# itxtx/normalizing-flows-study

Measured on AMD Instinct MI355X. Metric: log_prob samples/sec/GPU + test-NLL match; RealNVP d=2 and MAF d=63, higher is better.
Workload: dtype fp32

## Files before the change

### normalizing-flows-study_amd/csrc/nfx_affine.hip

```cpp
#include <atomic>
#include <climits>
#include <cstdlib>

#include "nfx_affine_kernel.h"
#include "nfx_affine_small_kernel.h"
#include "nfx_pack.h"

namespace nfx {


__global__ void affine_pack_kernel(NfxMlpRaw s_net, NfxMlpRaw b_net, const float* mask, int d,
                                   int H, float* packed) {
    const int HT = (H + 31) / 32;
    const AffineLayout L = affine_layout(d, HT);
    for (int i = blockIdx.x * blockDim.x + threadIdx.x; i < L.s; i += gridDim.x * blockDim.x) {
        float v = 0.f;
        if (i >= L.mask) {
            int j = i - L.mask;
            v = j < d ? mask[j] : 0.f;
        } else {
            const int net = i / L.net;
            const NfxMlpRaw& P = net ? b_net : s_net;
            const int o = i - net * L.net;
            if (o < L.b1) {
                const RowCol e = a1_elem(o - L.w1, L.KS1);
                v = (e.row < H && e.col < d) ? mlp_weight(P, 0, d, e.row, e.col) : 0.f;
            } else if (o < L.w2) {
                int row = acc_vec_row(o - L.b1);
                v = row < H ? mlp_bias(P, 0, row) : 0.f;
            } else if (o < L.b2) {
                const ATileElem e = a_tile_elem(o - L.w2);
                int row = 32 * (e.tile / HT) + e.row, col = 32 * (e.tile % HT) + e.k;
                v = (row < H && col < H) ? mlp_weight(P, 1, H, row, col) : 0.f;
            } else if (o < L.w3) {
                int row = acc_vec_row(o - L.b2);
                v = row < H ? mlp_bias(P, 1, row) : 0.f;
            } else if (o < L.b3 && d > 8) {
                const ATileElem e = a_tile_elem(o - L.w3);
                int row = 32 * (e.tile / HT) + e.row, col = 32 * (e.tile % HT) + e.k;
                v = (row < d && col < H) ? mlp_weight(P, 2, H, row, col) : 0.f;
            } else if (o < L.b3) {
                int t = o - L.w3, j = t / (32 * HT), col = acc_vec_row(t % (32 * HT));
                v = col < H ? mlp_weight(P, 2, H, j, col) : 0.f;
            } else if (d > 8) {
                int row = acc_vec_row(o - L.b3);
                v = row < d ? mlp_bias(P, 2, row) : 0.f;
            } else {
                int j = o - L.b3;
                v = j < d ? mlp_bias(P, 2, j) : 0.f;
            }
        }
        packed[i] = v;
    }
}

__global__ __launch_bounds__(1024) void affine_split_pack_kernel(float* packed, int d, int H) {
    const int HT = (H + 31) / 32, KS1 = (d + 1) / 2;
    const AffineLayout L = affine_layout(d, HT);
    const AffineSplit S = affine_split(d, HT);
    float* out = packed + L.s;
    __shared__ int w2_bad;
    __shared__ float rowsum[2 * 64], bmax[2 * 64], w2sum[2 * 64], w3sum[2 * 8];
    if (threadIdx.x == 0) w2_bad = 0;
    __syncthreads();
    bool bad = false;
    for (int i = threadIdx.x; i < S.total; i += blockDim.x) {
        const int net = i < S.mask ? i / S.net : 0;
        const int o = i - net * S.net;
        const float* P = packed + net * L.net;
        uint32_t v = 0;
        if (i >= S.ok) {
            continue;
        } else if (i >= S.mask) {
            v = __float_as_uint(packed[L.mask + (i - S.mask)]);
        } else if (o < S.b1) {
            v = __float_as_uint(P[L.w1 + (o - S.w1)]);
        } else if (o < S.b2) {
            v = __float_as_uint(P[L.b1 + (o - S.b1)]);
        } else if (o < S.w3) {
            v = __float_as_uint(P[L.b2 + (o - S.b2)]);
        } else if (o < S.b3) {
            v = __float_as_uint(P[L.w3 + (o - S.w3)]);
        } else if (o < S.w2s) {
            v = __float_as_uint(P[L.b3 + (o - S.b3)]);
        } else {
            const int t = o - S.w2s, q = t & 3, lane = (t >> 2) & 63, g = t >> 8;
            const int p = g % 3, kb = (g / 3) % (2 * HT), hto = (g / 3) / (2 * HT);
            const int kt = kb >> 1;
            uint32_t half[2];
            for (int e = 0; e < 2; ++e) {
                const int r = 8 * (kb & 1) + 2 * q + e;
                const float w = P[L.w2 + ((hto * HT + kt) * 4 + (r >> 2)) * 256 + lane * 4 + (r & 3)];
                if (!(fabsf(w) <= 1e6f)) bad = true;
                const uint32_t u0 = __builtin_bit_cast(uint16_t, (__bf16)w);
                const float r1 = w - __uint_as_float(u0 << 16);
                const uint32_t u1 = __builtin_bit_cast(uint16_t, (__bf16)r1);
                const uint32_t u2 = __builtin_bit_cast(uint16_t, (__bf16)(r1 - __uint_as_float(u1 << 16)));
                half[e] = p == 0 ? u0 : p == 1 ? u1 : u2;
            }
            v = half[0] | (half[1] << 16);
        }
        out[i] = __uint_as_float(v);
    }
    if (bad) atomicOr(&w2_bad, 1);
    for (int i = threadIdx.x; i < 2 * 64; i += blockDim.x) {
        rowsum[i] = 0.f;
        bmax[i] = 0.f;
        w2sum[i] = 0.f;
        if (i < 2 * 8) w3sum[i] = 0.f;
    }
    __syncthreads();
    if (threadIdx.x < 2 * 32 * HT) {
        const int net = threadIdx.x / (32 * HT), row = threadIdx.x % (32 * HT), ht = row >> 5, c = row & 31;
        const float* P = packed + net * L.net;
        float sum = 0.f;
        for (int ks = 0; ks < KS1; ++ks)
            for (int hh = 0; hh < 2; ++hh) sum += fabsf(P[L.w1 + (ht * KS1 + ks) * 64 + c + 32 * hh]);
        rowsum[net * 64 + row] = sum;
        float b = 0.f;
        for (int r = 0; r < 16; ++r)
            for (int hh = 0; hh < 2; ++hh)
                if (crow(r, hh) == c) b = fabsf(P[L.b1 + ht * 32 + 16 * hh + r]);
        bmax[net * 64 + row] = b;
        float s2 = 0.f;
        for (int g = 0; g < HT * 4; ++g)
            for (int hh = 0; hh < 2; ++hh)
                for (int rr = 0; rr < 4; ++rr) s2 += fabsf(P[L.w2 + (ht * HT * 4 + g) * 256 + (c + 32 * hh) * 4 + rr]);
        w2sum[net * 64 + row] = s2;
    }
    if (threadIdx.x < 2 * d) {
        const int net = threadIdx.x / d, j = threadIdx.x % d;
        const float* P = packed + net * L.net;
        float s3 = 0.f;
        for (int t = 0; t < HT * 32; ++t) s3 += fabsf(P[L.w3 + j * HT * 32 + t]);
        w3sum[net * 8 + j] = s3;
    }
    __syncthreads();
    if (threadIdx.x == 0) {
        float n1 = 0.f, c1 = 0.f;
        bool nan = false;
        for (int i = 0; i < 2 * 64; ++i) {
            nan = nan || !(rowsum[i] <= 3e38f) || !(bmax[i] <= 3e38f);
            n1 = fmaxf(n1, rowsum[i]);
            c1 = fmaxf(c1, bmax[i]);
        }
        const float xs = nan ? 0.f : (1e30f - c1) / n1;
        bool lost = false;
        for (int net = 0; net < 2; ++net) {
            float r2 = 0.f, r3 = 0.f;
            for (int i = 0; i < 64; ++i) r2 = fmaxf(r2, w2sum[net * 64 + i]);
            for (int j = 0; j < 8; ++j) r3 = fmaxf(r3, w3sum[net * 8 + j]);
            lost = lost || !(0x1p-133 * (double)r2 * (double)r3 < 0x1p-24);
        }
        out[S.ok] = (w2_bad || lost) ? 0.f : 1.f;
        out[S.ok + 1] = xs > 0.f ? xs : 0.f;
        out[S.ok + 2] = 0.f;
        out[S.ok + 3] = 0.f;
    }
}

int affine_split_pack(float* packed, int d, int H, hipStream_t s) {
    if (!affine_has_split(d, (H + 31) / 32)) return NFX_OK;
    affine_split_pack_kernel<<<1, 1024, 0, s>>>(packed, d, H);
    return check_launch("affine_split_pack_kernel");
}

static affine_kernel_t pick_affine(int HT, int d, int dir, bool logp) {
    return pick_range<1, 4>(HT, [=](auto HT_) { return affine_pick_ht<HT_()>(d, dir, logp); });
}

static affine_kernel_t pick_affine_small(int HT, int d, int dir, bool logp) {
    return pick_range<1, 4>(HT, [=](auto HT_) { return affine_small_pick_ht<HT_()>(d, dir, logp); });
}

static std::atomic<int>& affine_policy() {
    static std::atomic<int> v{[] {
        const char* e = getenv("NFX_AFFINE_POLICY");
        return e ? atoi(e) : NFX_AFFINE_AUTO;
    }()};
    return v;
}

int affine_policy_get() { return affine_policy().load(std::memory_order_relaxed); }

typedef void (*affine_wide_t)(const float*, const float*, float*, float*, int64_t, int, int, int64_t, float*,
                              double*, double*, float);

template <int HT>
static affine_wide_t wide_pick(int dir, bool logp) {
    if (dir > 0) return affine_wide_kernel<HT, 1, false>;
    return logp ? affine_wide_kernel<HT, -1, true> : affine_wide_kernel<HT, -1, false>;
}

static int affine_wide_launch(const float* packed, const float* in, float* out, float* log_det, int64_t B, int d,
                              int H, int direction, int accumulate, float* logp, double* sums, void* workspace,
                              hipStream_t stream) {
    const bool fused = sums != nullptr;
    const int HT = (H + 31) / 32;
    if (d > 64 || HT > 4)
        return set_error(NFX_EUNSUPPORTED, "affine_coupling: d=%d H=%d outside the compiled family (d<=64, H<=128)", d, H);
    affine_wide_t k = pick_range<1, 4>(HT, [=](auto HT_) { return wide_pick<HT_()>(direction, fused); });
    if (B == 0) return fused ? gauss_finish(reinterpret_cast<double*>(workspace), 0, sums, 0, stream) : NFX_OK;
    if (!packed || !in || !out || !log_det) return set_error(NFX_EINVAL, "affine_coupling: null pointer");
    if (in == out) return set_error(NFX_EINVAL, "affine_coupling: in and out must not alias");
    const size_t lds = (size_t)kWideWaves * 32 * (d | 1) * sizeof(float);
    const int64_t ntiles = (B + 31) / 32;
    int grid = resident_grid((const void*)k, 64 * kWideWaves, lds, (ntiles + kWideWaves - 1) / kWideWaves);
    if (grid > kMaxPartials) grid = kMaxPartials;
    double* partials = reinterpret_cast<double*>(workspace);
    k<<<grid, 64 * kWideWaves, lds, stream>>>(packed, in, out, log_det, B, d, accumulate, ntiles, logp, partials,
                                              sums, gauss_const(d));
    return check_launch("affine_wide_kernel");
}

static int affine_launch(const float* packed, const float* in, float* out, float* log_det, int64_t B,
                         int d, int H, int direction, int accumulate, float* logp, double* sums,
// ... 111 lines not shown
```

### normalizing-flows-study_amd/csrc/nfx_affine_kernel.h

```cpp
#pragma once
#include <type_traits>
#include <utility>

#include "nfx_common.h"

namespace nfx {

__host__ __device__ constexpr int up4(int v) { return (v + 3) & ~3; }

struct AffineLayout {
    int d, HT, KS1;
    int w1, b1, w2, b2, w3, b3, net, mask, total;
    int s;
};

struct AffineSplit {
    int w1, b1, b2, w3, b3, w2s, net, mask, ok, total;
};

__host__ __device__ constexpr AffineSplit affine_split(int d, int HT) {
    AffineSplit S{};
    int o = 0;
    S.w1 = o; o += HT * ((d + 1) / 2) * 64;
    S.b1 = o; o += HT * 32;
    S.b2 = o; o += HT * 32;
    S.w3 = o; o += d * HT * 32;
    S.b3 = o; o += up4(d);
    S.w2s = o; o += HT * 2 * HT * 768;
    S.net = o;
    S.mask = 2 * o;
    S.ok = S.mask + up4(d);
    S.total = S.ok + 4;
    return S;
}

__host__ __device__ constexpr bool affine_has_split(int d, int HT) { return d <= 8 && HT <= 2; }

__host__ __device__ constexpr AffineLayout affine_layout(int d, int HT) {
    AffineLayout L{};
    L.d = d;
    L.HT = HT;
    L.KS1 = (d + 1) / 2;
    int o = 0;
    L.w1 = o; o += HT * L.KS1 * 64;
    L.b1 = o; o += HT * 32;
    L.w2 = o; o += HT * HT * 16 * 64;
    L.b2 = o; o += HT * 32;
    if (d <= 8) {
        L.w3 = o; o += d * HT * 32;
        L.b3 = o; o += up4(d);
    } else {
        const int NJ = (d + 31) / 32;
        L.w3 = o; o += NJ * HT * 1024;
        L.b3 = o; o += NJ * 32;
    }
    L.net = o;
    L.mask = 2 * o;
    L.total = 2 * o + up4(d);
    L.s = L.total;
    if (affine_has_split(d, HT)) L.total += affine_split(d, HT).total;
    return L;
}

template <int D>
__device__ __forceinline__ void load_row(const float* __restrict__ p, float (&v)[D]) {
    if constexpr (D == 2) {
        float2 t = *reinterpret_cast<const float2*>(p);
        v[0] = t.x; v[1] = t.y;
// ... 78 lines not shown
    for (int j = 0; j < D; ++j)
        res[j] = tclamp(halves_sum(part[j][0], part[j][1]) + P[L.b3 + j], -10.f, 10.f);
}

#ifndef NFX_SPLIT_TERMS
#define NFX_SPLIT_TERMS 6
#endif
typedef __bf16 bf16x8 __attribute__((ext_vector_type(8)));
typedef uint32_t u32x4 __attribute__((ext_vector_type(4)));

__device__ __forceinline__ f32x16 mfma_bf16(u32x4 a, u32x4 b, f32x16 c) {
    return __builtin_amdgcn_mfma_f32_32x32x16_bf16(__builtin_bit_cast(bf16x8, a), __builtin_bit_cast(bf16x8, b), c,
                                                    0, 0, 0);
}

__device__ __forceinline__ void split3(float x, uint32_t& u0, uint32_t& u1, uint32_t& u2) {
    u0 = __float_as_uint(x) & 0xffff0000u;
    const float r1 = x - __uint_as_float(u0);
    u1 = __float_as_uint(r1) & 0xffff0000u;
    u2 = __float_as_uint(r1 - __uint_as_float(u1));
}

__device__ __forceinline__ uint32_t pack_bf16(uint32_t lo, uint32_t hi) {
    return __builtin_amdgcn_perm(hi, lo, 0x07060302u);
}

__device__ __forceinline__ void split_block(const f32x16& a, int half, u32x4 (&xp)[3]) {
#pragma unroll
    for (int q = 0; q < 4; ++q) {
        uint32_t l0, l1, l2, h0, h1, h2;
        split3(a[8 * half + 2 * q], l0, l1, l2);
        split3(a[8 * half + 2 * q + 1], h0, h1, h2);
        xp[0][q] = pack_bf16(l0, h0);
        xp[1][q] = pack_bf16(l1, h1);
        xp[2][q] = pack_bf16(l2, h2);
    }
}

template <class F, int... I>
__device__ __forceinline__ void static_for_seq(F&& f, std::integer_sequence<int, I...>) {
    (f(std::integral_constant<int, I>{}), ...);
}
template <int N, class F>
__device__ __forceinline__ void static_for(F&& f) {
    static_for_seq(f, std::make_integer_sequence<int, N>{});
}

#if NFX_SPLIT_TERMS == 8
constexpr int kSplitTermW[8] = {2, 1, 2, 1, 0, 1, 0, 0}, kSplitTermX[8] = {1, 2, 0, 1, 2, 0, 1, 0};
#else
constexpr int kSplitTermW[6] = {2, 1, 0, 1, 0, 0}, kSplitTermX[6] = {0, 1, 2, 0, 1, 0};
#endif

template <int HT, int D, int TILES>
__device__ __forceinline__ void affine_nets_split_pipe(const float* __restrict__ S, const AffineSplit& SL,
                                                       const float (&xb)[2][(D + 1) / 2], float (&sv)[D],
                                                       float (&bv)[D]) {
    constexpr int KS1 = (D + 1) / 2;
    constexpr int NS = 2 * TILES;
    constexpr int KB = 2 * HT;
    constexpr int NT = NFX_SPLIT_TERMS;
    constexpr int NM = NT * HT;
    constexpr int NG = KB * NM;
    constexpr int NFI = 16 * HT;
    constexpr int NQ = 3 * HT;
    constexpr int WG0 = (NM - NQ) / 2;
    constexpr int L1G = (KB - 2) * NM;
    constexpr int L1P = L1G >= 2 ? L1G - 2 : 0;
    constexpr int HB0 = NM / 2;
    const int lane = lane_id(), h = lane >> 5;

    const float* Sn[NS];
    const u32x4* w2n[NS];
    f32x16 h1[NS][HT];
    uint32_t u[NS * KB][3][8];
    u32x4 xp[NS * KB][3];
    u32x4 w[NS * KB][HT][3];
    f32x16 hi[NS][HT], lo[NS][HT];
    f32x4 w3q[NS][HT][D][4];
    float r1[NS * KB][8], tf[NS][NFI];
    float part[2][D][2];
#pragma unroll
    for (int n = 0; n < 2; ++n)
#pragma unroll
        for (int j = 0; j < D; ++j) part[n][j][0] = part[n][j][1] = 0.f;

    auto base = [&](int s) __attribute__((always_inline)) {
        Sn[s] = S + (s / TILES) * SL.net + opaque_zero();
        w2n[s] = reinterpret_cast<const u32x4*>(Sn[s] + SL.w2s) + lane;
    };
    auto l1_bias = [&](int s) __attribute__((always_inline)) {
#pragma unroll
        for (int ht = 0; ht < HT; ++ht) h1[s][ht] = load_bias16(Sn[s] + SL.b1 + ht * 32, h);
    };
    auto l1_mfma = [&](int s) __attribute__((always_inline)) {
#pragma unroll
        for (int ht = 0; ht < HT; ++ht)
#pragma unroll
            for (int ks = 0; ks < KS1; ++ks)
                h1[s][ht] = mfma32(Sn[s][SL.w1 + (ht * KS1 + ks) * 64 + lane], xb[s % TILES][ks], h1[s][ht]);
    };
    auto split_slot = [&](int b, int i) __attribute__((always_inline)) {
        const int s = b / KB, kb = b % KB, q = i / 3;
#pragma unroll
        for (int e = 2 * q; e < 2 * q + 2; ++e) {
            if (i % 3 == 0) {
                const float x = trelu(h1[s][kb >> 1][8 * (kb & 1) + e]);
                u[b][0][e] = __float_as_uint(x) & 0xffff0000u;
                r1[b][e] = x - __uint_as_float(u[b][0][e]);
            } else if (i % 3 == 1) {
                u[b][1][e] = __float_as_uint(r1[b][e]) & 0xffff0000u;
                u[b][2][e] = __float_as_uint(r1[b][e] - __uint_as_float(u[b][1][e]));
            }
        }
        if (i % 3 == 2) {
#pragma unroll
            for (int p = 0; p < 3; ++p) xp[b][p][q] = pack_bf16(u[b][p][2 * q], u[b][p][2 * q + 1]);
        }
    };
    auto w2_quad = [&](int b, int i) __attribute__((always_inline)) {
        const int s = b / KB, kb = b % KB, p = 2 - i / HT, hto = i % HT;
        w[b][hto][p] = w2n[s][((hto * KB + kb) * 3 + p) * 64];
    };
    auto w3_quads = [&](int s, int hto, int rq) __attribute__((always_inline)) {
#pragma unroll
        for (int j = 0; j < D; ++j)
            w3q[s][hto][j][rq] = *reinterpret_cast<const f32x4*>(Sn[s] + SL.w3 + (j * HT + hto) * 32 + 16 * h + 4 * rq);
    };
    auto fold_relu = [&](int s, int f) __attribute__((always_inline)) {
        tf[s][f] = trelu(hi[s][f / 16][f % 16] + lo[s][f / 16][f % 16]);
    };
    auto fold_fma = [&](int s, int f) __attribute__((always_inline)) {
        const int hto = f / 16, r = f % 16;
#pragma unroll
        for (int j = 0; j < D; ++j)
            part[s / TILES][j][s % TILES] = fmaf(w3q[s][hto][j][r / 4][r % 4], tf[s][f], part[s / TILES][j][s % TILES]);
    };
    constexpr auto fold_gap = [](int f) { return (((f | 1) + 1) * NG + NFI - 1) / NFI - 1; };
    constexpr auto w3_gap = [](int f) {
        const int g = (((f | 1) + 1) * NG + NFI - 1) / NFI - 1;
        return g >= 2 ? g - 2 : 0;
    };
    static_assert(fold_gap(NFI - 1) < NG && fold_gap(0) >= 1 && w3_gap(0) < fold_gap(0), "fold schedule");
    static_assert(WG0 >= 0 && WG0 + NQ <= NM && HB0 + HT <= NM - HT, "read schedule");
    static_assert(KB < 2 || L1G <= (KB - 1) * NM - 1, "layer 1 of the next stage precedes its first split");

    base(0);
    l1_bias(0);
#pragma unroll
    for (int i = 0; i < NQ; ++i) w2_quad(0, i);
    l1_mfma(0);
#pragma unroll
    for (int i = 0; i < 12; ++i) split_slot(0, i);

    static_for<NS>([&](auto sc) __attribute__((always_inline)) {
        constexpr int s = decltype(sc)::value;
        static_for<NG>([&](auto gc) __attribute__((always_inline)) {
            constexpr int g = decltype(gc)::value;
            constexpr int kb = g / NM, m = g % NM, b = s * KB + kb;
            constexpr int t = m / HT, hto = m % HT;
            __builtin_amdgcn_sched_barrier(0);
            if (t == NT - 1) {
                hi[s][hto] = mfma_bf16(w[b][hto][kSplitTermW[t]], xp[b][kSplitTermX[t]], hi[s][hto]);
            } else {
                lo[s][hto] = mfma_bf16(w[b][hto][kSplitTermW[t]], xp[b][kSplitTermX[t]],
                                       kb == 0 && t == 0 ? f32x16{} : lo[s][hto]);
            }
            __builtin_amdgcn_sched_barrier(0);
            if (g == 0 && s + 1 < NS) base(s + 1);
            if (b + 1 < NS * KB && m >= WG0 && m < WG0 + NQ) w2_quad(b + 1, m - WG0);
            if (kb == 0 && m >= HB0 && m < HB0 + HT)
                hi[s][m - HB0] = load_bias16(Sn[s] + SL.b2 + (m - HB0) * 32, h);
            if (s > 0) {
#pragma unroll
                for (int fq = 0; fq < NFI; fq += 4)
                    if (w3_gap(fq) == g) w3_quads(s - 1, fq / 16, (fq % 16) / 4);
            }
            if (s + 1 < NS && g == L1P) l1_bias(s + 1);
            if (s + 1 < NS && g == L1G) l1_mfma(s + 1);
            if (b + 1 < NS * KB) {
#pragma unroll
                for (int i = m * 12 / NM; i < (m + 1) * 12 / NM; ++i) split_slot(b + 1, i);
            }
            if (s > 0) {
#pragma unroll
                for (int f = 0; f < NFI; ++f)
                    if ((fold_gap(f) >= 1 ? fold_gap(f) - 1 : 0) == g) fold_relu(s - 1, f);
#pragma unroll
                for (int f = 0; f < NFI; ++f)
                    if (fold_gap(f) == g) fold_fma(s - 1, f);
            }
        });
    });
    __builtin_amdgcn_sched_barrier(0);
#pragma unroll
    for (int fq = 0; fq < NFI; fq += 4) w3_quads(NS - 1, fq / 16, (fq % 16) / 4);
#pragma unroll
    for (int f = 0; f < NFI; ++f) {
        fold_relu(NS - 1, f);
        fold_fma(NS - 1, f);
    }
#pragma unroll
    for (int j = 0; j < D; ++j) {
        sv[j] = tclamp(halves_sum(part[0][j][0], part[0][j][1]) + Sn[0][SL.b3 + j], -10.f, 10.f);
        bv[j] = tclamp(halves_sum(part[1][j][0], part[1][j][1]) + Sn[NS - 1][SL.b3 + j], -10.f, 10.f);
    }
}

template <int HT, int D, int TILES = 2>
__device__ __forceinline__ void affine_net_split(const float* __restrict__ S, const AffineSplit& SL,
                                                 const float (&xb)[2][(D + 1) / 2], float (&res)[D]) {
    constexpr int KS1 = (D + 1) / 2;
    const int lane = lane_id(), h = lane >> 5;

    f32x16 h1[HT][2];
#pragma unroll
    for (int ht = 0; ht < HT; ++ht) {
        f32x16 a0, a1;
        load_bias16_x2(S + SL.b1 + ht * 32, h, a0, a1);
#pragma unroll
        for (int ks = 0; ks < KS1; ++ks) {
            const float w = S[SL.w1 + (ht * KS1 + ks) * 64 + lane];
            a0 = mfma32(w, xb[0][ks], a0);
            if constexpr (TILES == 2) a1 = mfma32(w, xb[1][ks], a1);
        }
#pragma unroll
        for (int r = 0; r < 16; ++r) {
            a0[r] = trelu(a0[r]);
            if constexpr (TILES == 2) a1[r] = trelu(a1[r]);
        }
        h1[ht][0] = a0;
        h1[ht][1] = a1;
    }

    float part[D][2];
#pragma unroll
    for (int j = 0; j < D; ++j) part[j][0] = part[j][1] = 0.f;
    auto fold = [&](int hto, const f32x16& a, int st) {
#pragma unroll
        for (int j = 0; j < D; ++j) {
            const f32x16 w3 = load_bias16(S + SL.w3 + (j * HT + hto) * 32, h);
#pragma unroll
            for (int r = 0; r < 16; ++r) part[j][st] = fmaf(w3[r], trelu(a[r]), part[j][st]);
        }
    };
    const u32x4* w2s = reinterpret_cast<const u32x4*>(S + SL.w2s) + lane;
#pragma unroll
    for (int st = 0; st < TILES; ++st) {
        u32x4 xp[2 * HT][3];
#pragma unroll
        for (int kb = 0; kb < 2 * HT; ++kb) split_block(h1[kb >> 1][st], kb & 1, xp[kb]);
        const u32x4* w2 = w2s + opaque_zero();
#pragma unroll
        for (int hto = 0; hto < HT; ++hto) {
            f32x16 hi = load_bias16(S + SL.b2 + hto * 32 + opaque_zero(), h), lo = {};
#pragma unroll
            for (int kb = 0; kb < 2 * HT; ++kb) {
                const int g = (hto * 2 * HT + kb) * 3;
                const u32x4 w[3] = {w2[g * 64], w2[(g + 1) * 64], w2[(g + 2) * 64]};
#if NFX_SPLIT_TERMS == 8
                lo = mfma_bf16(w[2], xp[kb][1], lo);
                lo = mfma_bf16(w[1], xp[kb][2], lo);
#endif
                lo = mfma_bf16(w[2], xp[kb][0], lo);
                lo = mfma_bf16(w[1], xp[kb][1], lo);
                lo = mfma_bf16(w[0], xp[kb][2], lo);
                lo = mfma_bf16(w[1], xp[kb][0], lo);
                lo = mfma_bf16(w[0], xp[kb][1], lo);
                hi = mfma_bf16(w[0], xp[kb][0], hi);
            }
            fold(hto, hi + lo, st);
        }
    }
#pragma unroll
    for (int j = 0; j < D; ++j)
        res[j] = tclamp(halves_sum(part[j][0], part[j][1]) + S[SL.b3 + j], -10.f, 10.f);
}

__host__ __device__ constexpr bool affine_split_piped(int HT, int D) { return HT == 2 && D <= 4; }

template <int HT, int D, int TILES, bool PIPE>
__device__ __forceinline__ void affine_nets_split(const float* __restrict__ S, const AffineSplit& SL,
                                                  const float* __restrict__ Pg, const AffineLayout& L,
                                                  const float (&xb)[2][(D + 1) / 2], float (&sv)[D], float (&bv)[D]) {
    constexpr int KS1 = (D + 1) / 2;
    const bool wok = S[SL.ok] != 0.f;
    const float xs = S[SL.ok + 1];
    bool fast[2];
#pragma unroll
    for (int st = 0; st < 2; ++st) {
        bool bad = false;
#pragma unroll
        for (int ks = 0; ks < KS1; ++ks) bad = bad || !(fabsf(xb[st][ks]) <= xs);
        fast[st] = wok && __builtin_amdgcn_ballot_w64(bad) == 0;
    }
    if constexpr (PIPE) {
        affine_nets_split_pipe<HT, D, TILES>(S, SL, xb, sv, bv);
    } else {
        affine_net_split<HT, D, TILES>(S, SL, xb, sv);
        __builtin_amdgcn_sched_barrier(0);
        affine_net_split<HT, D, TILES>(S + SL.net, SL, xb, bv);
    }
    if (!(fast[0] && (TILES == 1 || fast[1]))) {
        __builtin_amdgcn_sched_barrier(0);
        const float* P = Pg + opaque_zero();
        float s2[D], b2[D];
        affine_net<HT, D, TILES>(P, L, xb, s2);
        __builtin_amdgcn_sched_barrier(0);
        affine_net<HT, D, TILES>(P + L.net, L, xb, b2);
        if (!fast[lane_id() >> 5]) {
#pragma unroll
            for (int j = 0; j < D; ++j) {
                sv[j] = s2[j];
                bv[j] = b2[j];
            }
        }
    }
}

template <int HT, int D, int DIR, bool LOGP>
__global__ __launch_bounds__(256) void affine_coupling_kernel(
    const float* __restrict__ packed, const float* __restrict__ in, float* __restrict__ out,
    float* __restrict__ logdet, int64_t B, int accumulate, int64_t nchunks,
    float* __restrict__ logp, double* __restrict__ partials, double* __restrict__ sums, float cgauss) {
    constexpr AffineLayout L = affine_layout(D, HT);
    constexpr int KS1 = L.KS1;
    constexpr bool SPLIT = affine_has_split(D, HT);
    constexpr AffineSplit SL = affine_split(D, HT);
    constexpr int MASK = SPLIT ? SL.mask : L.mask;
    extern __shared__ f32x4 lds4[];
    {
        const f32x4* src = reinterpret_cast<const f32x4*>(packed + (SPLIT ? L.s : 0));
        for (int i = threadIdx.x; i < (SPLIT ? SL.total : L.total) / 4; i += 256) lds4[i] = src[i];
    }
    __syncthreads();
    const float* sm = reinterpret_cast<const float*>(lds4);

    const int lane = lane_id(), h = lane >> 5, col = lane & 31;
    const int64_t nwaves = (int64_t)gridDim.x * 4;
    float mk[D], mkb[KS1];
#pragma unroll
    for (int j = 0; j < D; ++j) mk[j] = sm[MASK + j];
#pragma unroll
    for (int ks = 0; ks < KS1; ++ks) mkb[ks] = (2 * ks + h < D) ? sm[MASK + 2 * ks + h] : 0.f;

    const int64_t wv = (int64_t)blockIdx.x * 4 + (threadIdx.x >> 6);
    const int64_t F = nchunks / nwaves, R = nchunks - F * nwaves;
    const bool split = 2 * R <= nwaves;
    const int64_t nfull = split ? F : F + (wv < R ? 1 : 0);
    const bool half = split && wv < 2 * R;
    const int64_t half_base = F * nwaves * 64 + wv * 32;

    struct Fetch {
        float xb[2][KS1];
        float xr[D];
        float ldin;
    };
    auto fetch = [&](int64_t u, Fetch& f) {
        const int64_t base = u < nfull ? (wv + u * nwaves) * 64 : half_base;
        const int nsamp = u < nfull ? 64 : (u == nfull && half ? 32 : 0);
#pragma unroll
        for (int st = 0; st < 2; ++st) {
            const int64_t s = base + 32 * st + col;
#pragma unroll
            for (int ks = 0; ks < KS1; ++ks) {
                const int k = 2 * ks + h;
                f.xb[st][ks] = (32 * st + col < nsamp && k < D && s < B) ? in[s * D + k] : 0.f;
            }
        }
        const int64_t so = base + lane;
        if (lane < nsamp && so < B) {
            load_row<D>(in + so * D, f.xr);
            f.ldin = accumulate ? logdet[so] : 0.f;
        } else {
#pragma unroll
            for (int j = 0; j < D; ++j) f.xr[j] = 0.f;
            f.ldin = 0.f;
        }
    };

    double lpacc = 0.0;
    auto unit = [&](auto tiles_c, int64_t base, const Fetch& cur) {
        constexpr int TILES = decltype(tiles_c)::value;
        const float* smi = sm + opaque_zero();
        float xb[2][KS1];
#pragma unroll
        for (int st = 0; st < 2; ++st) {
#pragma unroll
            for (int ks = 0; ks < KS1; ++ks) xb[st][ks] = cur.xb[st][ks] * mkb[ks];
        }

        float sv[D], bv[D];
        if constexpr (SPLIT) {
            affine_nets_split<HT, D, TILES, false>(smi, SL, packed, L, xb, sv, bv);
        } else {
            affine_net<HT, D, TILES>(smi, L, xb, sv);
            affine_net<HT, D, TILES>(smi + L.net, L, xb, bv);
        }
// ... 203 lines not shown
```

### normalizing-flows-study_amd/csrc/nfx_affine_schain.hip

```cpp
#include "nfx_chain.h"

namespace nfx {

template <int HT, int D>
__host__ __device__ constexpr int schain_wpad() {
    return (affine_split(D, HT).total + 255) & ~255;
}

template <int HT, int D, int DIR, bool LOGP, int NW>
__global__ __launch_bounds__(64 * NW) void affine_schain_kernel(
    NfxChainPacks packs, int nl, const float* __restrict__ in, float* __restrict__ out,
    float* __restrict__ logdet, int64_t B, int accumulate, int64_t nchunks, int slice_chunks,
    float* __restrict__ logp, double* __restrict__ partials, double* __restrict__ sums, float cgauss) {
    constexpr AffineLayout L = affine_layout(D, HT);
    constexpr AffineSplit SL = affine_split(D, HT);
    static_assert(affine_has_split(D, HT), "the streaming chain runs the split nets");
    constexpr int KS1 = L.KS1;
    constexpr int WPAD = schain_wpad<HT, D>();
    constexpr int NT = 64 * NW;
    extern __shared__ f32x4 lds4[];
    float* wbuf = reinterpret_cast<float*>(lds4);
    float* sx = wbuf + 2 * WPAD;
    float* sld = sx + (size_t)slice_chunks * 64 * D;

    const uint32_t wbuf_lds = lds_addr_of(lds4);
    const int wave = __builtin_amdgcn_readfirstlane(threadIdx.x >> 6);
    const int lane = lane_id(), h = lane >> 5, col = lane & 31;
    const int64_t c0 = nchunks * blockIdx.x / gridDim.x, c1 = nchunks * (blockIdx.x + 1) / gridDim.x;

    auto stage = [&](int li, int buf) {
        const float* src = packs.p[DIR > 0 ? li : nl - 1 - li] + L.s;
        for (int c = wave; c < WPAD / 256; c += NW) {
            int idx = c * 256 + lane * 4;
            if (idx > SL.total - 4) idx = SL.total - 4;
            lds_dma_x4(src + idx, wbuf_lds + (uint32_t)(buf * WPAD + c * 256) * 4u);
        }
    };

    double lpacc = 0.0;
    int g = 0;
    if (c0 < c1) stage(0, 0);
    for (int64_t s0 = c0; s0 < c1; s0 += slice_chunks) {
        const int64_t s1 = s0 + slice_chunks < c1 ? s0 + slice_chunks : c1;
        const int64_t r0 = s0 * 64;
        const int rows = (int)((B < s1 * 64 ? B : s1 * 64) - r0);
        for (int e = threadIdx.x; e < rows * D; e += NT) sx[e] = in[r0 * D + e];
        for (int e = threadIdx.x; e < rows; e += NT) sld[e] = accumulate ? logdet[r0 + e] : 0.f;
        const int nch = (int)(s1 - s0);
        const int F = nch / NW, R = nch - F * NW;
        const bool split = 2 * R <= NW;
        const int nfull = split ? F : F + (wave < R ? 1 : 0);
        const bool half = split && wave < 2 * R;
        const int half_base = F * NW * 64 + wave * 32;

        for (int li = 0; li < nl; ++li) {
            lds_dma_wait();
            __syncthreads();
            if (li + 1 < nl)
                stage(li + 1, (g + 1) & 1);
            else if (s0 + slice_chunks < c1)
                stage(0, (g + 1) & 1);
            const float* W = wbuf + (g & 1) * WPAD;
            const float* Pg = packs.p[DIR > 0 ? li : nl - 1 - li];
            const bool first = li == 0 && !accumulate;
            float mk[D], mkb[KS1];
#pragma unroll
            for (int j = 0; j < D; ++j) mk[j] = W[SL.mask + j];
#pragma unroll
            for (int ks = 0; ks < KS1; ++ks) mkb[ks] = (2 * ks + h < D) ? W[SL.mask + 2 * ks + h] : 0.f;

            auto unit = [&](auto tiles_c, int ub) {
                constexpr int TILES = decltype(tiles_c)::value;
                const int so = ub + lane;
                const bool act = lane < 32 * TILES && so < rows;
                float xr[D];
                if (act) {
                    load_row<D>(sx + so * D, xr);
                } else {
#pragma unroll
                    for (int j = 0; j < D; ++j) xr[j] = 0.f;
                }
                float xb[2][KS1];
                if constexpr (D == 2) {
                    const float other = halves_other(xr[0], xr[1]);
                    xb[0][0] = (h ? other : xr[0]) * mkb[0];
                    xb[1][0] = (h ? xr[1] : other) * mkb[0];
                } else {
#pragma unroll
                    for (int st = 0; st < 2; ++st) {
                        const int s = ub + 32 * st + col;
#pragma unroll
                        for (int ks = 0; ks < KS1; ++ks) {
                            const int k = 2 * ks + h;
                            xb[st][ks] = (32 * st + col < 32 * TILES && s < rows && k < D) ? sx[s * D + k] * mkb[ks] : 0.f;
                        }
                    }
                }
                const float* Wi = W + opaque_zero();
                float sv[D], bv[D];
                affine_nets_split<HT, D, TILES, affine_split_piped(HT, D)>(Wi, SL, Pg, L, xb, sv, bv);
                if (act) {
#pragma clang fp contract(off)
                    float y[D];
                    float ld = 0.f;
#pragma unroll
                    for (int j = 0; j < D; ++j) {
                        const float m = mk[j], om = 1.f - m;
                        const float xa = xr[j] * m;
                        float t;
                        if constexpr (DIR < 0) {
                            t = (xr[j] - bv[j]) * exp_fast(-sv[j]);
                            ld = ld + om * (-sv[j]);
                        } else {
                            t = xr[j] * exp_fast(sv[j]) + bv[j];
                            ld = ld + om * sv[j];
                        }
                        const float v = xa + om * t;
                        y[j] = nonfinite(v) ? 0.f : v;
                    }
                    if (nonfinite(ld)) ld = 0.f;
                    store_row<D>(sx + so * D, y);
                    sld[so] = first ? ld : sld[so] + ld;
                }
            };
            for (int u = 0; u < nfull; ++u) unit(std::integral_constant<int, 2>{}, (wave + u * NW) * 64);
            if (half) unit(std::integral_constant<int, 1>{}, half_base);
            ++g;
        }
        __syncthreads();
        for (int e = threadIdx.x; e < rows * D; e += NT) out[r0 * D + e] = sx[e];
        for (int e = threadIdx.x; e < rows; e += NT) {
            const float ldt = sld[e];
            logdet[r0 + e] = ldt;
            if constexpr (LOGP) {
                const float* rw = sx + (size_t)e * D;
                float m = gauss_sq0(rw[0]);
#pragma unroll
                for (int j = 1; j < D; ++j) m = gauss_sq(m, rw[j]);
                const float lp = gauss_lp(m, cgauss, ldt);
                logp[r0 + e] = lp;
                lpacc += (double)lp;
            }
        }
        __syncthreads();
    }
    if constexpr (LOGP) {
        logp_commit<NT>(lpacc, partials, sums, B);
    }
}

typedef void (*schain_t)(NfxChainPacks, int, const float*, float*, float*, int64_t, int, int64_t, int, float*,
                         double*, double*, float);

__host__ __device__ constexpr int schain_waves(int HT, int D) { return affine_split_piped(HT, D) ? 8 : 12; }

template <int HT, int D>
static schain_t schain_pick_d(int dir, bool logp) {
    constexpr int NW = schain_waves(HT, D);
    if (dir > 0) return affine_schain_kernel<HT, D, 1, false, NW>;
    return logp ? affine_schain_kernel<HT, D, -1, true, NW> : affine_schain_kernel<HT, D, -1, false, NW>;
}

static schain_t schain_pick(int HT, int D, int dir, bool logp) {
    if (HT == 1) return D == 2 ? schain_pick_d<1, 2>(dir, logp) : D == 4 ? schain_pick_d<1, 4>(dir, logp) : schain_pick_d<1, 8>(dir, logp);
    if (HT == 2) return D == 2 ? schain_pick_d<2, 2>(dir, logp) : D == 4 ? schain_pick_d<2, 4>(dir, logp) : schain_pick_d<2, 8>(dir, logp);
    return nullptr;
}

static int schain_wpad_rt(int HT, int D) {
    return (affine_split(D, HT).total + 255) & ~255;
}

constexpr size_t kSchainLds = 160 * 1024;
constexpr size_t kSchainStatic = 1024;

static int64_t schain_slice_cap(int HT, int D) {
    const size_t w = 2 * (size_t)schain_wpad_rt(HT, D) * sizeof(float);
    if (w + kSchainStatic >= kSchainLds) return 0;
    return (int64_t)((kSchainLds - kSchainStatic - w) / (64 * (D + 1) * sizeof(float)));
// ... 34 lines not shown
```

### normalizing-flows-study_amd/csrc/nfx_chain.h

```cpp
#pragma once
#include "nfx_affine_kernel.h"
#include "nfx_rng.h"

namespace nfx {

constexpr int kChainMax = 64;
struct NfxChainPacks {
    const float* p[kChainMax];
};

__device__ __forceinline__ void lds_dma_x4(const float* src, uint32_t lds_addr) {
    const uint32_t m = lds_addr;
    uint32_t keep;
    asm volatile(
        "s_mov_b32 %0, m0\n\t"
        "s_mov_b32 m0, %2\n\t"
        "s_nop 0\n\t"
        "global_load_lds_dwordx4 %1, off\n\t"
        "s_mov_b32 m0, %0"
        : "=&s"(keep)
        : "v"(src), "s"(__builtin_amdgcn_readfirstlane(m))
        : "memory");
}
template <typename T>
__device__ __forceinline__ uint32_t lds_addr_of(T* shared_array) {
    return (uint32_t)(uintptr_t)((__attribute__((address_space(3))) T*)shared_array);
}
__device__ __forceinline__ void lds_dma_wait() { asm volatile("s_waitcnt vmcnt(0)" ::: "memory"); }


int schain_launch(const NfxChainPacks& P, int nl, const float* in, float* out, float* log_det, int64_t B, int d,
                  int H, int direction, int accumulate, float* logp, double* sums, void* workspace, hipStream_t s);
bool schain_supported(int64_t B, int d, int H);
int affine_policy_get();
constexpr int64_t kSmallChainMaxB = 1 << 16;

}
```

### normalizing-flows-study_amd/csrc/nfx_spline_schain_kernel.h

```cpp
#pragma once
#include "nfx_chain.h"
#include "nfx_spline_kernel.h"

namespace nfx {

template <int HT>
__host__ __device__ constexpr int spline_schain_wpad() {
    return (spline_layout(HT, 2).total + 255) & ~255;
}

template <int HT, int K, int DIR, bool LOGP, int NW>
__global__ __launch_bounds__(64 * NW) void spline_schain_kernel(
    NfxChainPacks packs, int nl, const float* __restrict__ in, float* __restrict__ out,
    float* __restrict__ logdet, int64_t B, SplineConsts C, int accumulate, int64_t nchunks, int slice_chunks,
    float* __restrict__ logp, double* __restrict__ partials, double* __restrict__ sums, float cgauss,
    uint64_t seed, uint64_t* rng, float* __restrict__ zout) {
#pragma clang fp contract(off)
    constexpr int D = 2;
    constexpr SplineLayout L = spline_layout(HT, D);
    constexpr int WPAD = spline_schain_wpad<HT>();
    constexpr int NTH = 64 * NW;
    extern __shared__ f32x4 lds4[];
    float* wbuf = reinterpret_cast<float*>(lds4);
    float* sx = wbuf + 2 * WPAD;
    float* sld = sx + (size_t)slice_chunks * 64 * D;

    const uint32_t wbuf_lds = lds_addr_of(lds4);
    const int wave = __builtin_amdgcn_readfirstlane(threadIdx.x >> 6);
    const int lane = lane_id(), h = lane >> 5;
    const int64_t c0 = nchunks * blockIdx.x / gridDim.x, c1 = nchunks * (blockIdx.x + 1) / gridDim.x;

    auto stage = [&](int li, int buf) {
        const float* src = packs.p[DIR > 0 ? li : nl - 1 - li];
        for (int c = wave; c < WPAD / 256; c += NW) {
            int idx = c * 256 + lane * 4;
            if (idx > L.total - 4) idx = L.total - 4;
            lds_dma_x4(src + idx, wbuf_lds + (uint32_t)(buf * WPAD + c * 256) * 4u);
        }
    };

#ifdef NFX_SCHAIN_TIMING
    long long tacc[6] = {0, 0, 0, 0, 0, 0};
    long long tmark = clock64();
#define NFX_CMARK(k) do { const long long t_ = clock64(); tacc[k] += t_ - tmark; tmark = t_; } while (0)
#else
#define NFX_CMARK(k) do { } while (0)
#endif
    double lpacc = 0.0;
    int g = 0;
    if (c0 < c1) stage(0, 0);
    for (int64_t s0 = c0; s0 < c1; s0 += slice_chunks) {
        const int64_t s1 = s0 + slice_chunks < c1 ? s0 + slice_chunks : c1;
        const int64_t r0 = s0 * 64;
        const int rows = (int)((B < s1 * 64 ? B : s1 * 64) - r0);
        if (rng) {
            const uint64_t off = rng_offset(rng);
            for (int e = threadIdx.x; e < rows; e += NTH) {
                float z[D];
                base_draw<D>(r0 + e, seed, off, z);
                sx[e * D] = z[0];
                sx[e * D + 1] = z[1];
                if (zout) {
                    zout[(r0 + e) * D] = z[0];
                    zout[(r0 + e) * D + 1] = z[1];
                }
            }
        } else {
            for (int e = threadIdx.x; e < rows * D; e += NTH) sx[e] = in[r0 * D + e];
        }
        for (int e = threadIdx.x; e < rows; e += NTH) sld[e] = accumulate ? logdet[r0 + e] : 0.f;
        const int nch = (int)(s1 - s0);
        const int F = nch / NW, R = nch - F * NW;
        const bool split = 2 * R <= NW;
        const int nfull = split ? F : F + (wave < R ? 1 : 0);
        const bool half = split && wave < 2 * R;
        const int half_base = F * NW * 64 + wave * 32;

        NFX_CMARK(4);
        for (int li = 0; li < nl; ++li) {
            NFX_CMARK(3);
            lds_dma_wait();
            __syncthreads();
            NFX_CMARK(0);
            if (li + 1 < nl)
                stage(li + 1, (g + 1) & 1);
            else if (s0 + slice_chunks < c1)
                stage(0, (g + 1) & 1);
            const float* W = wbuf + (g & 1) * WPAD;
            const bool first = li == 0 && !accumulate;
            const int NT = (int)W[L.meta];
            const float mkb = h < D ? W[L.mask + h] : 0.f;

            auto unit = [&](auto tiles_c, int ub) {
                constexpr int TILES = decltype(tiles_c)::value;
                const int so = ub + lane;
                const bool act = lane < 32 * TILES && so < rows;
                float xr[D];
                if (act) {
                    const f32x2 v = *reinterpret_cast<const f32x2*>(sx + so * D);
                    xr[0] = v.x;
                    xr[1] = v.y;
                } else {
                    xr[0] = xr[1] = 0.f;
                }
                float xb[2][4];
                {
                    const float other = halves_other(xr[0], xr[1]);
                    float xraw[2] = {h ? other : xr[0], h ? xr[1] : other};
#pragma unroll
                    for (int st = 0; st < 2; ++st) {
                        float xv = xraw[st];
                        if (C.rescale) xv = C.rs_to_scale * (xv - C.rs_lo) - C.bound;
                        xb[st][0] = xv * mkb;
                        xb[st][1] = xb[st][2] = xb[st][3] = 0.f;
                    }
                }
                float y[D];
                float ld;
#ifdef NFX_SCHAIN_TIMING
                {
                    const float* Wz = W + opaque_zero();
                    f32x16 h2[HT][2];
                    spline_unit_hidden<HT, TILES>(Wz, L, 1, xb, h2);
                    float prm[32];
                    spline_unit_params<HT, TILES>(Wz, L, h2, 0, prm);
                    NFX_CMARK(1);
#pragma unroll
                    for (int j = 0; j < D; ++j) y[j] = xr[j];
                    ld = 0.f;
                    spline_unit_dim<K, DIR, D>(C, (int)Wz[L.tdim], 0, prm, xr, y, ld);
                    NFX_CMARK(2);
                }
#else
                if constexpr (NW > 8 && HT > 1)
                    spline_unit_apply_tseq<HT, K, DIR, D, TILES>(W + opaque_zero(), L, C, 1, NT, xb, xr, y, ld);
                else
                    spline_unit_apply<HT, K, DIR, D, TILES>(W + opaque_zero(), L, C, 1, NT, xb, xr, y, ld);
#endif
                if (act) {
                    float yo[D];
#pragma unroll
                    for (int j = 0; j < D; ++j) yo[j] = nonfinite(y[j]) ? 0.f : y[j];
                    *reinterpret_cast<f32x2*>(sx + so * D) = f32x2{yo[0], yo[1]};
                    if (nonfinite(ld)) ld = 0.f;
                    sld[so] = first ? ld : sld[so] + ld;
                }
            };
            for (int u = 0; u < nfull; ++u) unit(std::integral_constant<int, 2>{}, (wave + u * NW) * 64);
            if (half) unit(std::integral_constant<int, 1>{}, half_base);
            ++g;
        }
        NFX_CMARK(3);
        __syncthreads();
        for (int e = threadIdx.x; e < rows * D; e += NTH) out[r0 * D + e] = sx[e];
        for (int e = threadIdx.x; e < rows; e += NTH) {
            const float ldt = sld[e];
            logdet[r0 + e] = ldt;
            if constexpr (LOGP) {
                const float* rw = sx + (size_t)e * D;
                const float m = gauss_sq(gauss_sq0(rw[0]), rw[1]);
                const float lp = gauss_lp(m, cgauss, ldt);
                logp[r0 + e] = lp;
                lpacc += (double)lp;
            }
        }
        __syncthreads();
    }
    NFX_CMARK(5);
#ifdef NFX_SCHAIN_TIMING
    if (blockIdx.x == 0 && lane == 0 && (wave == 0 || wave == 4))
        for (int k = 0; k < 6; ++k) out[(wave ? 6 : 0) + k] = (float)tacc[k];
#endif
    if constexpr (LOGP) {
        logp_commit<NTH>(lpacc, partials, sums, B);
    }
    if (rng) rng_commit(rng);
}

typedef void (*spline_schain_t)(NfxChainPacks, int, const float*, float*, float*, int64_t, SplineConsts, int, int64_t,
                                int, float*, double*, double*, float, uint64_t, uint64_t*, float*);

constexpr int kSplineSchainWaves = 12;
constexpr int kSplineSchainWavesSmall = 8;

template <int HT>
spline_schain_t spline_schain_pick_ht(int K, int dir, bool logp, bool small);

template <int HT, int K, int NW>
spline_schain_t spline_schain_dir(int dir, bool logp) {
    if (dir > 0) return spline_schain_kernel<HT, K, 1, false, NW>;
    return logp ? spline_schain_kernel<HT, K, -1, true, NW> : spline_schain_kernel<HT, K, -1, false, NW>;
}

template <int HT>
spline_schain_t spline_schain_pick(int K, int dir, bool logp, bool small) {
    return pick_range<kSplineMinK, kSplineMaxK>(K, [=](auto K_) {
        return small ? spline_schain_dir<HT, K_(), kSplineSchainWavesSmall>(dir, logp)
                     : spline_schain_dir<HT, K_(), kSplineSchainWaves>(dir, logp);
    });
}

}
// ... 1 lines not shown
```

Measured before the change: 1.578 billion.

## Elide masked-out output rows in affine split pipe and rebalance chain tiles per SIMD

The pack kernel now detects which coupling-layer outputs are masked (their s/b are discarded) and, when numerically safe, records a compact list of live output indices. The piped split-net kernel then computes only the live half of the final-layer outputs, which cuts w3 loads, registers and FMAs, with a ballot-based fallback to the full path when the inputs look unsafe. Separately, the leftover-chunk distribution in the affine and spline chain kernels is reworked so extra tiles are spread evenly across the four SIMDs, backed by compile-time ownership checks. This adds another kernel instantiation and code size, and the fallback check costs extra work when it fires.

```diff
diff --git a/normalizing-flows-study_amd/csrc/nfx_affine.hip b/normalizing-flows-study_amd/csrc/nfx_affine.hip
--- a/normalizing-flows-study_amd/csrc/nfx_affine.hip
+++ b/normalizing-flows-study_amd/csrc/nfx_affine.hip
@@ -54,7 +54,7 @@
     }
 }
 
-__global__ __launch_bounds__(1024) void affine_split_pack_kernel(float* packed, int d, int H) {
+__global__ __launch_bounds__(1024) void affine_split_pack_kernel(float* packed, int d, int H, int live_fold) {
     const int HT = (H + 31) / 32, KS1 = (d + 1) / 2;
     const AffineLayout L = affine_layout(d, HT);
     const AffineSplit S = affine_split(d, HT);
@@ -152,16 +152,38 @@
             for (int j = 0; j < 8; ++j) r3 = fmaxf(r3, w3sum[net * 8 + j]);
             lost = lost || !(0x1p-133 * (double)r2 * (double)r3 < 0x1p-24);
         }
-        out[S.ok] = (w2_bad || lost) ? 0.f : 1.f;
+        const bool wok = !(w2_bad || lost);
+        out[S.ok] = wok ? 1.f : 0.f;
         out[S.ok + 1] = xs > 0.f ? xs : 0.f;
-        out[S.ok + 2] = 0.f;
-        out[S.ok + 3] = 0.f;
+        int nlive = 0;
+        uint32_t idx = 0x88888888u;
+        bool dead_ok = wok && xs > 0.f && live_fold;
+        for (int j = 0; j < d; ++j) {
+            if (packed[L.mask + j] == 1.0f) {
+                for (int net = 0; net < 2; ++net) {
+                    const float* P = packed + net * L.net;
+                    float r2 = 0.f, b2 = 0.f;
+                    for (int i = 0; i < 64; ++i) r2 = fmaxf(r2, w2sum[net * 64 + i]);
+                    for (int i = 0; i < HT * 32; ++i) b2 = fmaxf(b2, fabsf(P[L.b2 + i]));
+                    const double hmax = 1e30 * (double)r2 + (double)b2;
+                    dead_ok = dead_ok && (double)w3sum[net * 8 + j] * hmax + (double)fabsf(P[L.b3 + j]) <= 1e37;
+                }
+            } else {
+                if (nlive < 8) idx = (idx & ~(0xfu << (4 * nlive))) | ((uint32_t)j << (4 * nlive));
+                ++nlive;
+                if (w3sum[j] == 0.f && packed[L.b3 + j] == 0.f) dead_ok = false;
+            }
+        }
+        const bool elide = dead_ok && nlive >= 1 && nlive <= (d + 1) / 2;
+        out[S.ok + 2] = __uint_as_float((uint32_t)nlive | (elide ? kAffineLiveElide : 0u));
+        out[S.ok + 3] = __uint_as_float(idx);
     }
 }
 
 int affine_split_pack(float* packed, int d, int H, hipStream_t s) {
     if (!affine_has_split(d, (H + 31) / 32)) return NFX_OK;
-    affine_split_pack_kernel<<<1, 1024, 0, s>>>(packed, d, H);
+    const char* e = getenv("NFX_AFFINE_LIVE_FOLD");
+    affine_split_pack_kernel<<<1, 1024, 0, s>>>(packed, d, H, e && atoi(e) == 0 ? 0 : 1);
     return check_launch("affine_split_pack_kernel");
 }
 
diff --git a/normalizing-flows-study_amd/csrc/nfx_affine_kernel.h b/normalizing-flows-study_amd/csrc/nfx_affine_kernel.h
--- a/normalizing-flows-study_amd/csrc/nfx_affine_kernel.h
+++ b/normalizing-flows-study_amd/csrc/nfx_affine_kernel.h
@@ -14,6 +14,7 @@
     int s;
 };
 
+constexpr uint32_t kAffineLiveElide = 0x100u;
 struct AffineSplit {
     int w1, b1, b2, w3, b3, w2s, net, mask, ok, total;
 };
@@ -198,11 +199,12 @@
 constexpr int kSplitTermW[6] = {2, 1, 0, 1, 0, 0}, kSplitTermX[6] = {0, 1, 2, 0, 1, 0};
 #endif
 
-template <int HT, int D, int TILES>
+template <int HT, int D, int TILES, bool LIVE>
 __device__ __forceinline__ void affine_nets_split_pipe(const float* __restrict__ S, const AffineSplit& SL,
                                                        const float (&xb)[2][(D + 1) / 2], float (&sv)[D],
-                                                       float (&bv)[D]) {
+                                                       float (&bv)[D], uint32_t live_idx) {
     constexpr int KS1 = (D + 1) / 2;
+    constexpr int NJ = LIVE ? (D + 1) / 2 : D;
     constexpr int NS = 2 * TILES;
     constexpr int KB = 2 * HT;
     constexpr int NT = NFX_SPLIT_TERMS;
@@ -223,13 +225,16 @@
     u32x4 xp[NS * KB][3];
     u32x4 w[NS * KB][HT][3];
     f32x16 hi[NS][HT], lo[NS][HT];
-    f32x4 w3q[NS][HT][D][4];
+    f32x4 w3q[NS][HT][NJ][4];
     float r1[NS * KB][8], tf[NS][NFI];
-    float part[2][D][2];
+    float part[2][NJ][2];
+    int w3row[NJ];
+#pragma unroll
+    for (int j = 0; j < NJ; ++j) w3row[j] = (LIVE ? (int)((live_idx >> (4 * j)) & 7u) : j) * HT * 32;
 #pragma unroll
     for (int n = 0; n < 2; ++n)
 #pragma unroll
-        for (int j = 0; j < D; ++j) part[n][j][0] = part[n][j][1] = 0.f;
+        for (int j = 0; j < NJ; ++j) part[n][j][0] = part[n][j][1] = 0.f;
 
     auto base = [&](int s) __attribute__((always_inline)) {
         Sn[s] = S + (s / TILES) * SL.net + opaque_zero();
@@ -270,8 +275,8 @@
     };
     auto w3_quads = [&](int s, int hto, int rq) __attribute__((always_inline)) {
 #pragma unroll
-        for (int j = 0; j < D; ++j)
-            w3q[s][hto][j][rq] = *reinterpret_cast<const f32x4*>(Sn[s] + SL.w3 + (j * HT + hto) * 32 + 16 * h + 4 * rq);
+        for (int j = 0; j < NJ; ++j)
+            w3q[s][hto][j][rq] = *reinterpret_cast<const f32x4*>(Sn[s] + SL.w3 + w3row[j] + hto * 32 + 16 * h + 4 * rq);
     };
     auto fold_relu = [&](int s, int f) __attribute__((always_inline)) {
         tf[s][f] = trelu(hi[s][f / 16][f % 16] + lo[s][f / 16][f % 16]);
@@ -279,7 +284,7 @@
     auto fold_fma = [&](int s, int f) __attribute__((always_inline)) {
         const int hto = f / 16, r = f % 16;
 #pragma unroll
-        for (int j = 0; j < D; ++j)
+        for (int j = 0; j < NJ; ++j)
             part[s / TILES][j][s % TILES] = fmaf(w3q[s][hto][j][r / 4][r % 4], tf[s][f], part[s / TILES][j][s % TILES]);
     };
     constexpr auto fold_gap = [](int f) { return (((f | 1) + 1) * NG + NFI - 1) / NFI - 1; };
@@ -346,11 +351,38 @@
         fold_relu(NS - 1, f);
         fold_fma(NS - 1, f);
     }
-#pragma unroll
-    for (int j = 0; j < D; ++j) {
-        sv[j] = tclamp(halves_sum(part[0][j][0], part[0][j][1]) + Sn[0][SL.b3 + j], -10.f, 10.f);
-        bv[j] = tclamp(halves_sum(part[1][j][0], part[1][j][1]) + Sn[NS - 1][SL.b3 + j], -10.f, 10.f);
-    }
+    if constexpr (LIVE) {
+#pragma unroll
+        for (int j = 0; j < D; ++j) sv[j] = bv[j] = 0.f;
+#pragma unroll
+        for (int jj = 0; jj < NJ; ++jj) {
+            const int o = (int)((live_idx >> (4 * jj)) & 15u);
+            const float s = tclamp(halves_sum(part[0][jj][0], part[0][jj][1]) + Sn[0][SL.b3 + (o & 7)], -10.f, 10.f);
+            const float b = tclamp(halves_sum(part[1][jj][0], part[1][jj][1]) + Sn[NS - 1][SL.b3 + (o & 7)], -10.f, 10.f);
+#pragma unroll
+            for (int j = 0; j < D; ++j) {
+                sv[j] = o == j ? s : sv[j];
+                bv[j] = o == j ? b : bv[j];
+            }
+        }
+    } else {
+#pragma unroll
+        for (int j = 0; j < D; ++j) {
+            sv[j] = tclamp(halves_sum(part[0][j][0], part[0][j][1]) + Sn[0][SL.b3 + j], -10.f, 10.f);
+            bv[j] = tclamp(halves_sum(part[1][j][0], part[1][j][1]) + Sn[NS - 1][SL.b3 + j], -10.f, 10.f);
+        }
+    }
+}
+
+template <int KS1>
+__device__ __forceinline__ bool affine_live_unit(const float (&xb)[2][KS1], const float (&mkb)[KS1]) {
+    bool bad = false;
+#pragma unroll
+    for (int st = 0; st < 2; ++st)
+#pragma unroll
+        for (int ks = 0; ks < KS1; ++ks)
+            bad = bad || (mkb[ks] == 1.f && (!(fabsf(xb[st][ks]) <= 1e33f) || __float_as_uint(xb[st][ks]) == 0x80000000u));
+    return __builtin_amdgcn_ballot_w64(bad) == 0;
 }
 
 template <int HT, int D, int TILES = 2>
@@ -428,7 +460,8 @@
 template <int HT, int D, int TILES, bool PIPE>
 __device__ __forceinline__ void affine_nets_split(const float* __restrict__ S, const AffineSplit& SL,
                                                   const float* __restrict__ Pg, const AffineLayout& L,
-                                                  const float (&xb)[2][(D + 1) / 2], float (&sv)[D], float (&bv)[D]) {
+                                                  const float (&xb)[2][(D + 1) / 2], float (&sv)[D], float (&bv)[D],
+                                                  bool live = false, uint32_t live_idx = 0) {
     constexpr int KS1 = (D + 1) / 2;
     const bool wok = S[SL.ok] != 0.f;
     const float xs = S[SL.ok + 1];
@@ -441,7 +474,15 @@
         fast[st] = wok && __builtin_amdgcn_ballot_w64(bad) == 0;
     }
     if constexpr (PIPE) {
-        affine_nets_split_pipe<HT, D, TILES>(S, SL, xb, sv, bv);
+        bool full = !live;
+        if (live) {
+            affine_nets_split_pipe<HT, D, TILES, true>(S, SL, xb, sv, bv, live_idx);
+            bool zero = true;
+#pragma unroll
+            for (int j = 0; j < D; ++j) zero = zero && fabsf(sv[j]) < 1e-30f;
+            full = __builtin_amdgcn_ballot_w64(zero) != 0;
+        }
+        if (full) affine_nets_split_pipe<HT, D, TILES, false>(S, SL, xb, sv, bv, 0u);
     } else {
         affine_net_split<HT, D, TILES>(S, SL, xb, sv);
         __builtin_amdgcn_sched_barrier(0);
@@ -489,7 +530,6 @@
     for (int j = 0; j < D; ++j) mk[j] = sm[MASK + j];
 #pragma unroll
     for (int ks = 0; ks < KS1; ++ks) mkb[ks] = (2 * ks + h < D) ? sm[MASK + 2 * ks + h] : 0.f;
-
     const int64_t wv = (int64_t)blockIdx.x * 4 + (threadIdx.x >> 6);
     const int64_t F = nchunks / nwaves, R = nchunks - F * nwaves;
     const bool split = 2 * R <= nwaves;
diff --git a/normalizing-flows-study_amd/csrc/nfx_affine_schain.hip b/normalizing-flows-study_amd/csrc/nfx_affine_schain.hip
--- a/normalizing-flows-study_amd/csrc/nfx_affine_schain.hip
+++ b/normalizing-flows-study_amd/csrc/nfx_affine_schain.hip
@@ -47,11 +47,8 @@
         for (int e = threadIdx.x; e < rows * D; e += NT) sx[e] = in[r0 * D + e];
         for (int e = threadIdx.x; e < rows; e += NT) sld[e] = accumulate ? logdet[r0 + e] : 0.f;
         const int nch = (int)(s1 - s0);
-        const int F = nch / NW, R = nch - F * NW;
-        const bool split = 2 * R <= NW;
-        const int nfull = split ? F : F + (wave < R ? 1 : 0);
-        const bool half = split && wave < 2 * R;
-        const int half_base = F * NW * 64 + wave * 32;
+        const ChainShare share = chain_share(nch, NW, wave);
+        const int nwhole = share.nfull + (share.xtiles == 2 ? 1 : 0);
 
         for (int li = 0; li < nl; ++li) {
             lds_dma_wait();
@@ -68,6 +65,8 @@
             for (int j = 0; j < D; ++j) mk[j] = W[SL.mask + j];
 #pragma unroll
             for (int ks = 0; ks < KS1; ++ks) mkb[ks] = (2 * ks + h < D) ? W[SL.mask + 2 * ks + h] : 0.f;
+            [[maybe_unused]] const bool elide = (__builtin_amdgcn_readfirstlane(__float_as_uint(W[SL.ok + 2])) & kAffineLiveElide) != 0;
+            [[maybe_unused]] const uint32_t live_idx = __builtin_amdgcn_readfirstlane(__float_as_uint(W[SL.ok + 3]));
 
             auto unit = [&](auto tiles_c, int ub) {
                 constexpr int TILES = decltype(tiles_c)::value;
@@ -98,7 +97,12 @@
                 }
                 const float* Wi = W + opaque_zero();
                 float sv[D], bv[D];
-                affine_nets_split<HT, D, TILES, affine_split_piped(HT, D)>(Wi, SL, Pg, L, xb, sv, bv);
+                if constexpr (affine_split_piped(HT, D)) {
+                    const bool live = elide && affine_live_unit<KS1>(xb, mkb);
+                    affine_nets_split<HT, D, TILES, true>(Wi, SL, Pg, L, xb, sv, bv, live, live_idx);
+                } else {
+                    affine_nets_split<HT, D, TILES, false>(Wi, SL, Pg, L, xb, sv, bv);
+                }
                 if (act) {
 #pragma clang fp contract(off)
                     float y[D];
@@ -123,8 +127,9 @@
                     sld[so] = first ? ld : sld[so] + ld;
                 }
             };
-            for (int u = 0; u < nfull; ++u) unit(std::integral_constant<int, 2>{}, (wave + u * NW) * 64);
-            if (half) unit(std::integral_constant<int, 1>{}, half_base);
+            for (int u = 0; u < nwhole; ++u)
+                unit(std::integral_constant<int, 2>{}, u < share.nfull ? (wave + u * NW) * 64 : share.xbase);
+            if (share.xtiles == 1) unit(std::integral_constant<int, 1>{}, share.xbase);
             ++g;
         }
         __syncthreads();
diff --git a/normalizing-flows-study_amd/csrc/nfx_chain.h b/normalizing-flows-study_amd/csrc/nfx_chain.h
--- a/normalizing-flows-study_amd/csrc/nfx_chain.h
+++ b/normalizing-flows-study_amd/csrc/nfx_chain.h
@@ -29,6 +29,68 @@
 __device__ __forceinline__ void lds_dma_wait() { asm volatile("s_waitcnt vmcnt(0)" ::: "memory"); }
 
 
+struct ChainShare {
+    int nfull, xtiles, xbase;
+};
+
+__host__ __device__ constexpr int chain_extra_tiles(int R, int NW, int w) {
+    const int K = NW / 4, s = w & 3, i = w >> 2;
+    const int q = (2 * R) / 4 + (s < (2 * R) % 4 ? 1 : 0);
+    if (q <= K) return i < q ? 1 : 0;
+    return i < q - K ? 2 : 1;
+}
+
+__host__ __device__ constexpr ChainShare chain_share(int nch, int NW, int wave) {
+    const int F = nch / NW, R = nch - F * NW;
+    const int mine = chain_extra_tiles(R, NW, wave);
+    int wholes = 0, wholes_before = 0, halves_before = 0;
+    for (int w = 0; w < NW; ++w) {
+        const int e = chain_extra_tiles(R, NW, w);
+        wholes += e == 2;
+        wholes_before += e == 2 && w < wave;
+        halves_before += e == 1 && w < wave;
+    }
+    const int idx = mine == 2 ? 2 * wholes_before : 2 * wholes + halves_before;
+    return ChainShare{F, mine, F * NW * 64 + idx * 32};
+}
+
+__host__ __device__ constexpr bool chain_share_ok(int NW, int nch0, int nch1) {
+    for (int nch = nch0; nch <= nch1; ++nch) {
+        int load[4] = {0, 0, 0, 0};
+        unsigned long long seen[8] = {0, 0, 0, 0, 0, 0, 0, 0};
+        for (int w = 0; w < NW; ++w) {
+            const ChainShare c = chain_share(nch, NW, w);
+            load[w & 3] += 2 * c.nfull + c.xtiles;
+            for (int u = 0; u <= c.nfull; ++u) {
+                const int tiles = u < c.nfull ? 2 : c.xtiles;
+                const int base = u < c.nfull ? (w + u * NW) * 64 : c.xbase;
+                if (tiles == 2 && base % 64 != 0) return false;
+                for (int t = 0; t < tiles; ++t) {
+                    const int tile = base / 32 + t;
+                    if (base % 32 != 0 || tile >= 2 * nch || (seen[tile >> 6] >> (tile & 63) & 1)) return false;
+                    seen[tile >> 6] |= 1ull << (tile & 63);
+                }
+            }
+        }
+        for (int t = 0; t < 2 * nch; ++t)
+            if (!(seen[t >> 6] >> (t & 63) & 1)) return false;
+        for (int s = 0; s < 4; ++s)
+            if (load[s] > (2 * nch + 3) / 4) return false;
+    }
+    return true;
+}
+#define NFX_CHAIN_SHARE_CHECK(lo, hi)                                                    \
+    static_assert(chain_share_ok(8, lo, hi) && chain_share_ok(12, lo, hi),               \
+                  "chain_share: a tile unowned, owned twice, or a SIMD overloaded")
+NFX_CHAIN_SHARE_CHECK(1, 64);
+NFX_CHAIN_SHARE_CHECK(65, 112);
+NFX_CHAIN_SHARE_CHECK(113, 152);
+NFX_CHAIN_SHARE_CHECK(153, 184);
+NFX_CHAIN_SHARE_CHECK(185, 208);
+NFX_CHAIN_SHARE_CHECK(209, 232);
+NFX_CHAIN_SHARE_CHECK(233, 256);
+#undef NFX_CHAIN_SHARE_CHECK
+
 int schain_launch(const NfxChainPacks& P, int nl, const float* in, float* out, float* log_det, int64_t B, int d,
                   int H, int direction, int accumulate, float* logp, double* sums, void* workspace, hipStream_t s);
 bool schain_supported(int64_t B, int d, int H);
diff --git a/normalizing-flows-study_amd/csrc/nfx_spline_schain_kernel.h b/normalizing-flows-study_amd/csrc/nfx_spline_schain_kernel.h
--- a/normalizing-flows-study_amd/csrc/nfx_spline_schain_kernel.h
+++ b/normalizing-flows-study_amd/csrc/nfx_spline_schain_kernel.h
@@ -70,11 +70,8 @@
         }
         for (int e = threadIdx.x; e < rows; e += NTH) sld[e] = accumulate ? logdet[r0 + e] : 0.f;
         const int nch = (int)(s1 - s0);
-        const int F = nch / NW, R = nch - F * NW;
-        const bool split = 2 * R <= NW;
-        const int nfull = split ? F : F + (wave < R ? 1 : 0);
-        const bool half = split && wave < 2 * R;
-        const int half_base = F * NW * 64 + wave * 32;
+        const ChainShare share = chain_share(nch, NW, wave);
+        const int nwhole = share.nfull + (share.xtiles == 2 ? 1 : 0);
 
         NFX_CMARK(4);
         for (int li = 0; li < nl; ++li) {
@@ -146,8 +143,9 @@
                     sld[so] = first ? ld : sld[so] + ld;
                 }
             };
-            for (int u = 0; u < nfull; ++u) unit(std::integral_constant<int, 2>{}, (wave + u * NW) * 64);
-            if (half) unit(std::integral_constant<int, 1>{}, half_base);
+            for (int u = 0; u < nwhole; ++u)
+                unit(std::integral_constant<int, 2>{}, u < share.nfull ? (wave + u * NW) * 64 : share.xbase);
+            if (share.xtiles == 1) unit(std::integral_constant<int, 1>{}, share.xbase);
             ++g;
         }
         NFX_CMARK(3);
```

New measurement: 1.661 billion (median of 6 runs). +5.3%, better.
